# Changfei-Fu/RUMI-SLAM

Measured on AMD Instinct MI355X. Metric: frames/sec ORB extract+match, higher is better.
Workload: dtype u8; 1 GPU; ORB extract (640x480, 8-level pyramid, 1000 features/frame) + brute-force 256-bit Hamming match of consecutive frames (BASELINE.json configs[1]+[2]); scaling=n/a (one GPU), exchange=none

## Files before the change

include/rumi_testhooks.h:

```cpp
#ifndef RUMI_TESTHOOKS_H
#define RUMI_TESTHOOKS_H
#include <stdint.h>
#ifdef __cplusplus
extern "C" {
#endif

int rumi_hook_sort_like_std(uint32_t *keys, uint16_t *ids, int32_t n);
int rumi_hook_sort_device(uint32_t *keys, uint16_t *ids, int32_t n);
int rumi_hook_std_sort(uint32_t *keys, uint16_t *ids, int32_t n);

int rumi_hook_quadtree(const uint32_t *cand, int32_t n, int32_t minX, int32_t maxX, int32_t minY, int32_t maxY,
                       int32_t N, int32_t *out_idx, int32_t cap, int32_t *n_out);

float rumi_hook_sinf(float x);
float rumi_hook_cosf(float x);
float rumi_hook_fast_atan2(float y, float x);
int rumi_hook_cv_round(float v);
int rumi_hook_magic_div(int32_t idx, int32_t d);

struct RumiMatcher;
int rumi_hook_newpts_matches(struct RumiMatcher *m, int32_t n_neigh, int32_t n1, int32_t *matches);

#ifdef __cplusplus
}
#endif
#endif
```

rumi_slam_amd/capi.py:

```python
import ctypes as C
import os

import numpy as np

_HERE = os.path.dirname(os.path.abspath(__file__))
LIB_PATH = os.path.join(_HERE, "librumi_hip.so")

RUMI_OK, RUMI_E_INVALID, RUMI_E_NO_DEVICE, RUMI_E_CAPACITY, RUMI_E_EMPTY = 0, -1, -2, -3, -4

KP_DTYPE = np.dtype([("x", "<f4"), ("y", "<f4"), ("size", "<f4"), ("angle", "<f4"),
                     ("response", "<f4"), ("octave", "<i4"), ("class_id", "<i4")])
assert KP_DTYPE.itemsize == 28


class RumiOrbConfig(C.Structure):
    _fields_ = [("nfeatures", C.c_int32), ("scale_factor", C.c_float), ("nlevels", C.c_int32),
                ("ini_th_fast", C.c_int32), ("min_th_fast", C.c_int32), ("max_width", C.c_int32),
                ("max_height", C.c_int32), ("max_batch", C.c_int32), ("device", C.c_int32),
                ("host_threads", C.c_int32), ("blur_variant", C.c_int32)]


class RumiError(RuntimeError):
    def __init__(self, code, msg):
        super().__init__(f"rumi status {code}: {msg}")
# ... 77 lines not shown


def kfdb_lib():
    L = lib()
    if getattr(L, "_kfdb_ready", False):
        return L
    vp, i32, i64, u64 = C.c_void_p, C.c_int32, C.c_int64, C.c_uint64
    L.rumi_kfdb_create.argtypes = [vp, i32, i64, i32, C.POINTER(vp)]
    L.rumi_kfdb_destroy.argtypes = [vp]
    L.rumi_kfdb_destroy.restype = None
    L.rumi_kfdb_clear.argtypes = [vp]
    L.rumi_kfdb_size.argtypes = [vp]
    L.rumi_kfdb_next_seq.argtypes = [vp]
    L.rumi_kfdb_next_seq.restype = i64
    L.rumi_kfdb_max_batch.argtypes = [vp]
    L.rumi_kfdb_add.argtypes = [vp, i32, vp, vp, vp, vp, vp]
    L.rumi_kfdb_add_batch_device.argtypes = [vp, i32, vp, vp, vp, vp, vp, i32, vp]
    L.rumi_kfdb_bow.argtypes = [vp, u64, vp, vp, i32, C.POINTER(i32)]
    L.rumi_kfdb_erase.argtypes = [vp, i32, vp]
    L.rumi_kfdb_clear_map.argtypes = [vp, i32]
    L.rumi_kfdb_set_map_bad.argtypes = [vp, i32, i32]
    L.rumi_kfdb_set_maps.argtypes = [vp, i32, vp, vp]
    L.rumi_kfdb_set_bad.argtypes = [vp, i32, vp, vp]
    L.rumi_kfdb_set_covisibles.argtypes = [vp, i32, vp, vp]
    L.rumi_kfdb_score.argtypes = [vp, i32, i32, vp, vp, vp, vp, vp, vp, vp, vp, vp]
    L.rumi_kfdb_scored.argtypes = [vp, vp, vp]
    L.rumi_kfdb_select_reloc.argtypes = [vp, vp, vp, i64]
    L.rumi_kfdb_select_nbest.argtypes = [vp, vp, i32, vp, vp, vp, vp]
    L._kfdb_ready = True
    return L


HOOK_SYMBOLS = ["rumi_hook_sort_like_std", "rumi_hook_sort_device", "rumi_hook_std_sort", "rumi_hook_quadtree", "rumi_hook_sinf", "rumi_hook_cosf",
                "rumi_hook_fast_atan2", "rumi_hook_cv_round", "rumi_hook_magic_div", "rumi_hook_newpts_matches"]


def hooks():
    L = lib()
    if getattr(L, "_hooks_ready", False):
        return L
    vp, i32 = C.c_void_p, C.c_int32
    L.rumi_hook_sort_like_std.argtypes = [vp, vp, i32]
    L.rumi_hook_sort_device.argtypes = [vp, vp, i32]
    L.rumi_hook_std_sort.argtypes = [vp, vp, i32]
    L.rumi_hook_quadtree.argtypes = [vp, i32, i32, i32, i32, i32, i32, vp, i32, C.POINTER(i32)]
    for name in ("rumi_hook_sinf", "rumi_hook_cosf"):
        getattr(L, name).restype = C.c_float
        getattr(L, name).argtypes = [C.c_float]
    L.rumi_hook_fast_atan2.restype = C.c_float
    L.rumi_hook_fast_atan2.argtypes = [C.c_float, C.c_float]
    L.rumi_hook_cv_round.argtypes = [C.c_float]
    L.rumi_hook_magic_div.argtypes = [i32, i32]
    L._hooks_ready = True
    return L
```

rumi_slam_amd/csrc/orb_geom.h:

```cpp
#pragma once
#include <algorithm>
#include <cfloat>
#include <cmath>
#include <cstdint>
#include <vector>

namespace rumi {

constexpr int kPatchSize = 31;
constexpr int kHalfPatch = 15;
constexpr int kEdge = 19;
constexpr int kBorder = kEdge - 3;
constexpr int kMaxLevels = 16;
constexpr int kCellTileMax = 96;

inline int cv_round_host(double v) { return (int)std::lrint(v); }

#if defined(__HIPCC__)
#define RUMI_GEOM_HD __host__ __device__ inline
#else
#define RUMI_GEOM_HD inline
#endif
RUMI_GEOM_HD unsigned magic_of(unsigned d) { return (1u << 20) / d + 1u; }
RUMI_GEOM_HD int magic_div(int idx, unsigned M) { return (int)(((unsigned)idx * M) >> 20); }
// ... 55 lines not shown
inline bool make_geometry(const OrbTables &t, int w, int h, std::vector<LevelGeom> &g,
                          long long *arenaBytes, int *totalCells, int *totalCand, int *maxCellCand) {
    g.assign(t.nlevels, LevelGeom{});
    long long off = 0;
    int cells = 0, cand = 0, cellCand = 1;
    for (int l = 0; l < t.nlevels; l++) {
        LevelGeom &L = g[l];
        L.w = cv_round_host((float)w * t.invScale[l]);
        L.h = cv_round_host((float)h * t.invScale[l]);
        L.pitch = (L.w + 63) & ~63;
        L.off = off;
        off += (long long)L.pitch * L.h + 64;
        L.maxBX = L.w - kBorder; L.maxBY = L.h - kBorder;
        const float width = (float)(L.maxBX - kBorder), height = (float)(L.maxBY - kBorder);
        L.nCols = (int)(width / 35.f); L.nRows = (int)(height / 35.f);
        if (L.nCols <= 0 || L.nRows <= 0) return false;
        L.wCell = (int)std::ceil(width / L.nCols); L.hCell = (int)std::ceil(height / L.nRows);
        if (L.wCell + 6 > kCellTileMax || L.hCell + 6 > kCellTileMax) return false;
        L.cellBase = cells; L.nCells = L.nCols * L.nRows; cells += L.nCells;
        L.nfeat = t.featuresPerLevel[l];
        L.scale = t.scale[l];
        const int dw = L.maxBX - kBorder - 6, dh = L.maxBY - kBorder - 6;
        L.candBase = cand;
        L.candCap = std::min(65535, std::max(1, ((dw + 1) / 2) * ((dh + 1) / 2)));
        cand += L.candCap;
        cellCand = std::max(cellCand, ((L.wCell + 1) / 2) * ((L.hCell + 1) / 2));
        L.coefOff = 0;
    }
    *arenaBytes = (off + 255) & ~255LL;
    *totalCells = cells; *totalCand = cand; *maxCellCand = cellCand;
    return true;
}

inline void make_resize_axis(int srcN, int dstN, bool clampX, std::vector<int16_t> &ofs,
                             std::vector<int16_t> &taps, int *maxOut) {
    const double inv = (double)dstN / srcN, scale = 1. / inv;
    ofs.resize(dstN); taps.resize(dstN * 2);
    int dmax = dstN;
    for (int d = 0; d < dstN; d++) {
        float f = (float)((d + 0.5) * scale - 0.5);
        int s = (int)std::floor(f);
        f -= s;
        if (clampX) {
            if (s < 0) { f = 0; s = 0; }
            if (s + 1 >= srcN) {
                dmax = std::min(dmax, d);
                if (s >= srcN - 1) { f = 0; s = srcN - 1; }
            }
        }
        ofs[d] = (int16_t)s;
        taps[d * 2] = (int16_t)cv_round_host((1.f - f) * 2048.f);
        taps[d * 2 + 1] = (int16_t)cv_round_host(f * 2048.f);
    }
    *maxOut = dmax;
}

}
```

rumi_slam_amd/csrc/orb_kernels.hip:

```cpp
#include <hip/hip_runtime.h>

#include "orb_device.h"
#include "orb_math.h"

namespace rumi {

struct PatternF { float v[256 * 4]; };
constexpr PatternF make_pattern_f() {
    constexpr int8_t src[256 * 4] = {
#include "orb_pattern.inc"
    };
    PatternF p{};
    for (int i = 0; i < 256 * 4; i++) p.v[i] = (float)src[i];
    return p;
}
__constant__ PatternF c_patternF = make_pattern_f();

__device__ __forceinline__ unsigned xcd_swizzle(unsigned lin, unsigned total) {
    const unsigned q = total >> 3, r = total & 7, xcd = lin & 7;
    return (xcd < r ? xcd * (q + 1) : r * (q + 1) + (xcd - r) * q) + (lin >> 3);
}

struct __attribute__((packed)) U32 { uint32_t v; };
struct __attribute__((packed)) U64 { uint64_t v; };
constexpr int kPyrLevels = 8, kPyrWinPasses = 20;

__device__ __forceinline__ const uint8_t *level_base(const ImgSrc &s, const DevParams *P, int level, int frame,
                                                      int *pitch) {
    if (level == 0) {
        *pitch = s.l0Pitch;
        return s.l0 + (long long)frame * s.l0FrameStride;
    }
    *pitch = P->lv[level].pitch;
    return s.pyr + (long long)frame * P->arenaStride + P->lv[level].off;
}

__device__ __forceinline__ int reflect101(int i, int n) {
    if (n == 1) return 0;
    while (i < 0 || i >= n) i = i < 0 ? -i : 2 * (n - 1) - i;
    return i;
}

template <int kResizeRows>
__global__ __launch_bounds__(256) void k_resize(const DevParams *__restrict__ P, ImgSrc src,
                                                const int16_t *__restrict__ coef, const RowTap *__restrict__ rowTab, int level, int32_t *__restrict__ clearWord) {
    if (clearWord && (blockIdx.x | blockIdx.y | blockIdx.z | threadIdx.x) == 0) *clearWord = 0;
    const DevLevel &D = P->lv[level];
    const DevLevel &S = P->lv[level - 1];
    const unsigned wg = xcd_swizzle((blockIdx.z * gridDim.y + blockIdx.y) * gridDim.x + blockIdx.x, gridDim.x * gridDim.y * gridDim.z);
    const int bx = wg % gridDim.x, by = (wg / gridDim.x) % gridDim.y, frame = wg / (gridDim.x * gridDim.y);
    const int ox = (bx * 64 + (threadIdx.x & 63)) * 4;
    const int oyBase = (by * 4 + __builtin_amdgcn_readfirstlane(threadIdx.x >> 6)) * kResizeRows;
    if (ox >= D.w || oyBase >= D.h) return;
    int sp;
    const uint8_t *sb = level_base(src, P, level - 1, frame, &sp);
    uint8_t *dbase = src.pyr + (long long)frame * P->arenaStride + D.off + ox;
    const int16_t *xofs = coef + D.coefX, *xa = coef + D.coefXT;
    const uint8_t *r0p[kResizeRows], *r1p[kResizeRows];
    uint32_t bh0[kResizeRows], bh1[kResizeRows];
    bool live[kResizeRows], shared[kResizeRows];
#pragma unroll
    for (int r = 0; r < kResizeRows; r++) {
        const int oy = oyBase + r;
        live[r] = oy < D.h;
        const RowTap t = rowTab[D.rowTab + (live[r] ? oy : 0)];
        r0p[r] = sb + (long long)t.r0 * sp; r1p[r] = sb + (long long)t.r1 * sp;
        bh0[r] = t.bh0; bh1[r] = t.bh1;
        shared[r] = kResizeRows == 4 && r > 0 && r0p[r] == r1p[r - 1];
    }
    const int sx0 = xofs[ox];
    if (ox + 3 < D.xmaxFast && xofs[ox + 3] + 1 - sx0 <= 7) {
        const int wx0 = min(sx0, S.w - 8);
        const uint64_t ofs = reinterpret_cast<const U64 *>(xofs + ox)->v;
        const U64 *t8 = reinterpret_cast<const U64 *>(xa + 2 * ox);
        const uint64_t ta = t8[0].v, tb = t8[1].v;
        uint64_t s0[kResizeRows], s1[kResizeRows];
#pragma unroll
        for (int r = 0; r < kResizeRows; r++) {
            s0[r] = 0;
            if (!shared[r]) s0[r] = reinterpret_cast<const U64 *>(r0p[r] + wx0)->v;
            s1[r] = reinterpret_cast<const U64 *>(r1p[r] + wx0)->v;
        }
        typedef unsigned short v2u16 __attribute__((ext_vector_type(2)));
        uint32_t sel[4], tap[4];
#pragma unroll
        for (int i = 0; i < 4; i++) {
            const uint32_t k = (uint32_t)((int)(int16_t)(ofs >> (16 * i)) - wx0);
            sel[i] = k | 0x0c000c00u | ((k + 1u) << 16);
            const uint64_t tt = i < 2 ? ta : tb;
            tap[i] = (uint32_t)(tt >> (32 * (i & 1)));
        }
        uint32_t hPrev[4] = {0, 0, 0, 0};
#pragma unroll
        for (int r = 0; r < kResizeRows; r++) {
            uint32_t h0[4], h1[4];
            if (shared[r]) {
#pragma unroll
                for (int i = 0; i < 4; i++) h0[i] = hPrev[i];
            } else {
#pragma unroll
                for (int i = 0; i < 4; i++) {
                    const uint32_t p0 = __builtin_amdgcn_perm((uint32_t)(s0[r] >> 32), (uint32_t)s0[r], sel[i]);
                    h0[i] = __builtin_amdgcn_udot2(__builtin_bit_cast(v2u16, p0), __builtin_bit_cast(v2u16, tap[i]), 0u, false) >> 4;
                }
            }
            uint32_t packed = 0;
#pragma unroll
            for (int i = 0; i < 4; i++) {
                const uint32_t p1 = __builtin_amdgcn_perm((uint32_t)(s1[r] >> 32), (uint32_t)s1[r], sel[i]);
                h1[i] = __builtin_amdgcn_udot2(__builtin_bit_cast(v2u16, p1), __builtin_bit_cast(v2u16, tap[i]), 0u, false) >> 4;
                packed |= ((__umulhi(bh0[r], h0[i]) + __umulhi(bh1[r], h1[i]) + 2u) >> 2) << (8 * i);
                hPrev[i] = h1[i];
            }
            if (live[r]) *reinterpret_cast<uint32_t *>(dbase + (long long)(oyBase + r) * D.pitch) = packed;
        }
    } else {
        for (int r = 0; r < kResizeRows; r++) {
            if (!live[r]) continue;
            uint32_t packed = 0;
            for (int i = 0; i < 4 && ox + i < D.w; i++) {
                const int dx = ox + i;
                const int sx = xofs[dx];
                int q0, q1;
                if (dx < D.xmax) {
                    const int a0 = xa[dx * 2], a1 = xa[dx * 2 + 1];
                    q0 = r0p[r][sx] * a0 + r0p[r][sx + 1] * a1;
                    q1 = r1p[r][sx] * a0 + r1p[r][sx + 1] * a1;
                } else {
                    q0 = r0p[r][sx] * 2048;
                    q1 = r1p[r][sx] * 2048;
                }
                packed |= (uint32_t)(((((int)(bh0[r] >> 16) * (q0 >> 4)) >> 16) + (((int)(bh1[r] >> 16) * (q1 >> 4)) >> 16) + 2) >> 2) << (8 * i);
            }
            *reinterpret_cast<uint32_t *>(dbase + (long long)(oyBase + r) * D.pitch) = packed;
        }
    }
}

__global__ __launch_bounds__(256) void k_pyramid_tiles(const DevParams *__restrict__ P, ImgSrc src, const int16_t *__restrict__ coef,
                                                       const RowTap *__restrict__ rowTab, const PyrTile *__restrict__ tiles, int bufBytes,
                                                       int32_t *__restrict__ clearWord) {
    extern __shared__ __attribute__((aligned(16))) uint8_t pyrLds[];
    if (clearWord && (blockIdx.x | blockIdx.y | threadIdx.x) == 0) *clearWord = 0;
    const int frame = blockIdx.y, tid = threadIdx.x, nlevels = P->nlevels;
    uint8_t *A = pyrLds, *B = pyrLds + bufBytes;
    uint2 *tab = reinterpret_cast<uint2 *>(pyrLds + 2 * bufBytes);
    struct Lv { int x0, x1, y0, y1, coefX, coefXT, xmax, rowTab, pitch, pad; long long off; };
    __shared__ Lv sLv[kMaxLevels];
    if (tid < nlevels) {
        const PyrTile &T = tiles[blockIdx.x];
        const DevLevel &D = P->lv[tid];
        sLv[tid] = Lv{T.x0[tid], T.x1[tid], T.y0[tid], T.y1[tid], D.coefX, D.coefXT, D.xmax, D.rowTab, D.pitch, 0, D.off};
    }
    __syncthreads();
    int apitch;
// ... 501 lines not shown
    }
    if (tid == 0) sStart[nc] = total;
    int run = base + inc - sum;
    for (int k = 0; k < chunk; k++) {
        const int c = tid * chunk + k;
        if (c < nc) { sStart[c] = run; run += cnt[c]; }
    }
    __syncthreads();
    int32_t *ls = levelStart + (long long)frame * (kMaxLevels + 1);
    if (blockIdx.y == 0 && tid <= P->nlevels) {
        const int c = tid < P->nlevels ? P->lv[tid].cellBase : nc;
        ls[tid] = sStart[c];
    }
    if (blockIdx.y == 0 && tid < P->nlevels) {
        const int c0 = P->lv[tid].cellBase, c1 = c0 + P->lv[tid].nCells;
        if (sStart[c1] - sStart[c0] > P->lv[tid].candCap) atomicOr(errFlag, 16);
    }
    uint32_t *out = cand + (long long)frame * P->totalCand;
    const int nOut = min(sStart[nc], P->totalCand);
    const uint32_t *inBase = cellBuf + (long long)frame * nc * P->maxCellCand;
    for (int j = blockIdx.y * kCompactThreads + tid; j < nOut; j += kCompactThreads * gridDim.y) {
        int lo = 0, hi = nc;
        while (hi - lo > 1) {
            const int mid = (lo + hi) >> 1;
            if (sStart[mid] <= j) lo = mid; else hi = mid;
        }
        out[j] = inBase[(long long)lo * P->maxCellCand + (j - sStart[lo])];
    }
}

constexpr int kBlurRowsSmall = 16, kBlurRowsBatch = 64;

struct BlurGrid { int base[kMaxLevels + 1]; int gx[kMaxLevels]; int bw[kMaxLevels]; };
__device__ __forceinline__ uint32_t mad_u24(uint32_t a, uint32_t b, uint32_t c) {
    uint32_t r;
    asm("v_mad_u32_u24 %0, %1, %2, %3" : "=v"(r) : "v"(a), "v"(b), "v"(c));
    return r;
}
template <int VARIANT, int kBlurRows>
__device__ __forceinline__ void blur_body(const DevParams *__restrict__ P, const ImgSrc &src, const BlurGrid &G, unsigned bxg, unsigned gxg) {
    constexpr uint32_t kT2 = VARIANT ? 49u : 48u, kT3 = VARIANT ? 55u : 56u;
    const int lane = threadIdx.x & 63, wave = __builtin_amdgcn_readfirstlane(threadIdx.x >> 6);
    const unsigned wg = xcd_swizzle(blockIdx.y * gxg + bxg, gxg * gridDim.y);
    const int frame = wg / gxg, lin = wg % gxg;
    int level = 0;
    for (int l = 1; l < P->nlevels; l++)
        if (lin >= G.base[l]) level = l;
    const DevLevel &L = P->lv[level];
    const int bx = (lin - G.base[level]) % G.gx[level], by = (lin - G.base[level]) / G.gx[level];
    const int bw = G.bw[level];
    const int xa = bx * bw + lane * 4;
    const int y0 = (by * 4 + wave) * kBlurRows;
    if (y0 >= L.h) return;
    int pitch;
    const uint8_t *img = level_base(src, P, level, frame, &pitch);
    uint8_t *out = src.blur + (long long)frame * P->arenaStride + L.off;
    const int w = L.w, h = L.h;
    const int xLast = (w - 1) & ~3;
    const int xl = min(xa, xLast);
    const bool firstBlock = bx == 0;
    const bool edgeWave = bx * bw + bw + 4 > w;
    const bool produce = lane * 4 < bw && xa < w;
    uint32_t selA = 0x03020100u, selB = 0x07060504u;
    if (edgeWave && xa + 3 >= w && xa <= xLast + 4) {
#pragma unroll
        for (int i = 0; i < 4; i++) {
            const int x = xa + i;
            if (x < w) continue;
            const int sx = 2 * (w - 1) - x, d = (xa - (sx & ~3)) >> 2;
            const uint32_t a = (d == 1 ? 4u : 0u) + (uint32_t)(sx & 3);
            const uint32_t b = d == 0 ? 4u + (uint32_t)(sx & 3) : (uint32_t)i;
            selA = (selA & ~(0xFFu << (8 * i))) | (a << (8 * i));
            selB = (selB & ~(0xFFu << (8 * i))) | (b << (8 * i));
        }
    }
    int ring[7][4];
#pragma unroll
    for (int k = 0; k < 7; k++)
#pragma unroll
        for (int i = 0; i < 4; i++) ring[k][i] = 0;
    const int yEnd = min(y0 + kBlurRows, h), rEnd = yEnd + 3;
    uint8_t *orow = out + (long long)(y0 - 6) * L.pitch + xa - L.pitch;
    const int haloOff = lane == 0 ? (firstBlock ? 0 : -4) : (lane == 63 && !edgeWave && bw == 256 ? 4 : 0);
    uint32_t Cn[7], Hn[7];
    auto fetch = [&](int r, uint32_t &C, uint32_t &H) {
        const int rc = min(r, rEnd - 1);
        const int rr = rc < 0 ? -rc : (rc >= h ? 2 * (h - 1) - rc : rc);
        const uint8_t *row = img + (long long)rr * pitch + xl;
        C = *reinterpret_cast<const uint32_t *>(row);
        H = 0;
        if (haloOff) H = *reinterpret_cast<const uint32_t *>(row + haloOff);
    };
#pragma unroll
    for (int j = 0; j < 7; j++) fetch(y0 - 3 + j, Cn[j], Hn[j]);
    uint32_t Cm[7], Hm[7];
    auto walk7 = [&](const uint32_t (&Cc)[7], const uint32_t (&Hc)[7], int r0) {
#pragma unroll
        for (int j = 0; j < 7; j++) {
            const int r = r0 + j;
            if (r >= rEnd) break;
            orow += L.pitch;
            uint32_t C = Cc[j];
            if (edgeWave) {
                const uint32_t c1 = __shfl_up(C, 1), c2 = __shfl_up(c1, 1);
                C = __builtin_amdgcn_perm(C, __builtin_amdgcn_perm(c1, c2, selA), selB);
            }
            uint32_t Lw = __shfl_up(C, 1), Rw = __shfl_down(C, 1);
            if (lane == 0) Lw = firstBlock ? __builtin_amdgcn_perm(C, C, 0x01020300u) : Hc[j];
            if (lane == 63 && !edgeWave && bw == 256) Rw = Hc[j];
            constexpr uint32_t tA = 18u | (34u << 8) | (kT2 << 16) | (kT3 << 24), tB = kT2 | (34u << 8) | (18u << 16);
            const uint32_t A0 = __builtin_amdgcn_alignbyte(C, Lw, 1), A1 = __builtin_amdgcn_alignbyte(C, Lw, 2), A2 = __builtin_amdgcn_alignbyte(C, Lw, 3);
            const uint32_t B0 = __builtin_amdgcn_alignbyte(Rw, C, 1), B1 = __builtin_amdgcn_alignbyte(Rw, C, 2), B2 = __builtin_amdgcn_alignbyte(Rw, C, 3);
            ring[j][0] = (int)__builtin_amdgcn_udot4(B0, tB, __builtin_amdgcn_udot4(A0, tA, 0u, false), false);
            ring[j][1] = (int)__builtin_amdgcn_udot4(B1, tB, __builtin_amdgcn_udot4(A1, tA, 0u, false), false);
            ring[j][2] = (int)__builtin_amdgcn_udot4(B2, tB, __builtin_amdgcn_udot4(A2, tA, 0u, false), false);
            ring[j][3] = (int)__builtin_amdgcn_udot4(Rw, tB, __builtin_amdgcn_udot4(C, tA, 0u, false), false);
            const int y = r - 3;
            if (y >= y0 && produce) {
                uint32_t o[4];
#pragma unroll
                for (int i = 0; i < 4; i++) {
                    uint32_t acc = mad_u24(kT3, (uint32_t)ring[(j + 4) % 7][i], 32768u);
                    acc = mad_u24(kT2, (uint32_t)(ring[(j + 3) % 7][i] + ring[(j + 5) % 7][i]), acc);
                    acc = mad_u24(34u, (uint32_t)(ring[(j + 2) % 7][i] + ring[(j + 6) % 7][i]), acc);
                    acc = mad_u24(18u, (uint32_t)(ring[(j + 1) % 7][i] + ring[j][i]), acc);
                    if (VARIANT) acc = min(acc, 0x00FFFFFFu);
                    o[i] = acc;
                }
                const uint32_t p01 = __builtin_amdgcn_perm(o[1], o[0], 0x0c0c0602u), p23 = __builtin_amdgcn_perm(o[3], o[2], 0x06020c0cu);
                *reinterpret_cast<uint32_t *>(orow) = p01 | p23;
            }
        }
    };
    for (int r0 = y0 - 3; r0 < rEnd; r0 += 7) {
#pragma unroll
        for (int j = 0; j < 7; j++) Cm[j] = Cn[j], Hm[j] = Hn[j];
        if (r0 + 7 < rEnd) {
#pragma unroll
            for (int j = 0; j < 7; j++) fetch(r0 + 7 + j, Cn[j], Hn[j]);
        }
        walk7(Cm, Hm, r0);
    }
}
template <int VARIANT, int kBlurRows>
__global__ __launch_bounds__(256) void k_blur(const DevParams *__restrict__ P, ImgSrc src, BlurGrid G) {
    blur_body<VARIANT, kBlurRows>(P, src, G, blockIdx.x, gridDim.x);
}
template <int TPC, int VARIANT>
__global__ __launch_bounds__(256) void k_fast_blur(const DevParams *__restrict__ P, ImgSrc src, FastLds F, uint32_t *__restrict__ cellBuf,
                                                   int32_t *__restrict__ cellCnt, BlurGrid G, unsigned gxFast) {
    if (blockIdx.x < gxFast) fast_cells_body<TPC>(P, src, F, cellBuf, cellCnt, blockIdx.x, gxFast);
    else blur_body<VARIANT, kBlurRowsSmall>(P, src, G, blockIdx.x - gxFast, gridDim.x - gxFast);
}

__device__ __forceinline__ int half_wave_sum(int v) {
    v += __builtin_amdgcn_update_dpp(0, v, 0x111, 0xF, 0xF, false);
    v += __builtin_amdgcn_update_dpp(0, v, 0x112, 0xF, 0xF, false);
    v += __builtin_amdgcn_update_dpp(0, v, 0x114, 0xF, 0xF, false);
    v += __builtin_amdgcn_update_dpp(0, v, 0x118, 0xF, 0xF, false);
    v += __builtin_amdgcn_update_dpp(0, v, 0x142, 0xA, 0xF, false);
    const int lo = __builtin_amdgcn_readlane(v, 31), hi = __builtin_amdgcn_readlane(v, 63);
    return (threadIdx.x & 32) ? hi : lo;
}
__device__ __forceinline__ int wave_sum(int v) {
#pragma unroll
    for (int o = 32; o > 0; o >>= 1) v += __shfl_xor(v, o);
    return v;
}

constexpr int kDiscP = 48, kPatchP = 48;
constexpr int kKpPerWg = 8;

struct AssembleArgs {
    const uint32_t *selLevel; const int32_t *selLevelCnt; int selLevelCap, lap0, lap1;
    int32_t *counts; long long countsStride; int32_t *errFlag, *errMirror;
    uint32_t *selPackedOut, *selMetaOut; int32_t *selCountOut;
};
template <int kKpGroups, bool kAssemble>
__global__ __launch_bounds__(256, 7) void k_orient_desc(const DevParams *__restrict__ P, ImgSrc src,
                                                     const uint32_t *__restrict__ selPacked,
                                                     const uint32_t *__restrict__ selMeta,
                                                     const int32_t *__restrict__ selCount, int selCap,
                                                     RumiKeyPoint *__restrict__ kpOut, long long kpStride, uint8_t *__restrict__ descOut,
                                                     long long descStride, int outCap, AssembleArgs A) {
    static_assert(kDiscP == kPatchP, "the disc and the patch share their rows");
// ... 198 lines not shown
    uint32_t pkC = 0, mtC = 0, pkN = 0, mtN = 0;
    if (liveC) key_rec(kb, pkC, mtC);
    if (liveN && kKpGroups > 1) key_rec(kb + kKpPerWg, pkN, mtN);
    if (kKpGroups == 1) liveN = false;
    Staged S;
    fetch_disc(pkC, mtC, liveC, S);
    fetch_patch(pkC, mtC, liveC, S);
#pragma unroll
    for (int g = 0; g < kKpGroups; g++) {
        if (!__any(liveC)) break;
        OD_STAMP(0);
        stage_disc(liveC, S);
        OD_STAMP(1);
        const int k2 = kb + (g + 2) * kKpPerWg;
        const bool liveNN = g + 2 < kKpGroups && k2 < cnt;
        uint32_t pkNN = 0, mtNN = 0;
        if (liveNN) key_rec(k2, pkNN, mtNN);
        if (g + 1 < kKpGroups) fetch_disc(pkN, mtN, liveN, S);
        OD_STAMP(2);
        float angle = 0.f;
        if (liveC) angle = orientation(pkC);
        stage_patch(liveC, S);
        if (g + 1 < kKpGroups) fetch_patch(pkN, mtN, liveN, S);
        if (liveC) describe(pkC, mtC, angle);
        OD_STAMP(3);
        pkC = pkN; mtC = mtN; liveC = liveN;
        pkN = pkNN; mtN = mtNN; liveN = liveNN;
    }
#ifdef RUMI_OD_STAMP
    if (threadIdx.x == 0 && (blockIdx.x % 8) == 0 && blockIdx.y == 0) printf("od wg %d: loop-head %lld stage(wait loads) %lld issue-next %lld | IC_Angle %lld trig %lld rBRIEF %lld store %lld\n", (int)blockIdx.x, st[0], st[1], st[2], st[4], st[5], st[6], st[3]);
#endif
}

void launch_resize(const DevParams *dP, const DevParams &hP, ImgSrc src, const int16_t *coef, const RowTap *rowTab, int level, int nframes,
                   hipStream_t st, int32_t *clearWord) {
    const int rows = hP.lv[level].h >= 200 ? 8 : 4;
    dim3 g((hP.lv[level].w + 255) / 256, (hP.lv[level].h + 4 * rows - 1) / (4 * rows), nframes);
    if (rows == 8) hipLaunchKernelGGL(k_resize<8>, g, dim3(256), 0, st, dP, src, coef, rowTab, level, clearWord);
    else hipLaunchKernelGGL(k_resize<4>, g, dim3(256), 0, st, dP, src, coef, rowTab, level, clearWord);
}
void launch_pyramid_tiles(const DevParams *dP, ImgSrc src, const int16_t *coef, const RowTap *rowTab, const PyrTile *tiles, int ntiles, int bufBytes,
                          int tabEntries, int nframes, hipStream_t st, int32_t *clearWord) {
    hipLaunchKernelGGL(k_pyramid_tiles, dim3(ntiles, nframes), dim3(256), (size_t)2 * bufBytes + (size_t)tabEntries * 8, st, dP, src, coef, rowTab, tiles, bufBytes, clearWord);
}
static FastLds fast_lds_of(const DevParams &hP) {
    int wMax = 0, hMax = 0;
    for (int l = 0; l < hP.nlevels; l++) { wMax = std::max(wMax, hP.lv[l].wCell); hMax = std::max(hMax, hP.lv[l].hCell); }
    FastLds F;
    F.tp = 4 * (((wMax + 3) >> 2) + 2);
    F.sp = F.tp;
    F.tileBytes = (hMax + 6) * F.tp;
    F.scBytes = ((hMax + 2) * F.sp + 15) & ~15;
    F.maxIters = (wMax * hMax + 63) / 64 + 1;
    F.tileBytes = (F.tileBytes + 15) & ~15;
    F.perWave = (F.tileBytes + F.scBytes + std::max(kRingCap * 2, F.maxIters * 8) + kScoredCap * 2 + 15) & ~15;
    return F;
}
void launch_fast(const DevParams *dP, const DevParams &hP, ImgSrc src, uint32_t *cellBuf, int32_t *cellCnt, int nframes,
                 hipStream_t st) {
    const FastLds F = fast_lds_of(hP);
    const int wpg = 4;
    const dim3 grid((hP.totalCells + wpg - 1) / wpg, nframes);
    const size_t lds = (size_t)wpg * F.perWave;
#define RUMI_FAST_CASE(T)                                                                                      \
    if (F.tp == T) {                                                                                           \
        hipLaunchKernelGGL((k_fast_cells<T>), grid, dim3(64 * wpg), lds, st, dP, src, F, cellBuf, cellCnt);    \
        return;                                                                                                \
    }
    RUMI_FAST_CASE(48) RUMI_FAST_CASE(44) RUMI_FAST_CASE(52) RUMI_FAST_CASE(56)
#undef RUMI_FAST_CASE
    hipLaunchKernelGGL((k_fast_cells<0>), grid, dim3(64 * wpg), lds, st, dP, src, F, cellBuf, cellCnt);
}
// ... 9 lines not shown
        const bool partialInFirstLanes = r >= 1 && r <= 8;
        const bool lane63Halo = bw == 256 && (r >= 253 || r <= 3);
        if (!partialInFirstLanes && !lane63Halo) return bw;
    }
    return 192;
}
static BlurGrid blur_grid_of(const DevParams &hP, int rows, int *total) {
    BlurGrid G{};
    int run = 0;
    for (int l = 0; l < hP.nlevels; l++) {
        G.bw[l] = blur_strip_width(hP.lv[l].w);
        G.gx[l] = (hP.lv[l].w + G.bw[l] - 1) / G.bw[l];
        G.base[l] = run;
        run += G.gx[l] * ((hP.lv[l].h + 4 * rows - 1) / (4 * rows));
    }
    G.base[hP.nlevels] = run;
    *total = run;
    return G;
}
bool fast_blur_fusable(const DevParams &hP) { return fast_lds_of(hP).tp == 48; }
bool launch_fast_blur(const DevParams *dP, const DevParams &hP, ImgSrc src, uint32_t *cellBuf, int32_t *cellCnt, int nframes, int variant, hipStream_t st) {
    const FastLds F = fast_lds_of(hP);
    if (F.tp != 48) return false;
    int run = 0;
    const BlurGrid G = blur_grid_of(hP, kBlurRowsSmall, &run);
    const int wpg = 4;
    const unsigned gxFast = (unsigned)((hP.totalCells + wpg - 1) / wpg);
    const dim3 grid(gxFast + (unsigned)run, nframes);
    const size_t lds = (size_t)wpg * F.perWave;
    if (variant) hipLaunchKernelGGL((k_fast_blur<48, 1>), grid, dim3(256), lds, st, dP, src, F, cellBuf, cellCnt, G, gxFast);
    else hipLaunchKernelGGL((k_fast_blur<48, 0>), grid, dim3(256), lds, st, dP, src, F, cellBuf, cellCnt, G, gxFast);
    return true;
}
void launch_blur(const DevParams *dP, const DevParams &hP, ImgSrc src, int nframes, int variant, hipStream_t st) {
    const bool small = nframes < 16;
    const int rows = small ? kBlurRowsSmall : kBlurRowsBatch;
    int run = 0;
    const BlurGrid G = blur_grid_of(hP, rows, &run);
    if (small) {
        if (variant) hipLaunchKernelGGL((k_blur<1, kBlurRowsSmall>), dim3(run, nframes), dim3(256), 0, st, dP, src, G);
        else hipLaunchKernelGGL((k_blur<0, kBlurRowsSmall>), dim3(run, nframes), dim3(256), 0, st, dP, src, G);
    } else {
        if (variant) hipLaunchKernelGGL((k_blur<1, kBlurRowsBatch>), dim3(run, nframes), dim3(256), 0, st, dP, src, G);
        else hipLaunchKernelGGL((k_blur<0, kBlurRowsBatch>), dim3(run, nframes), dim3(256), 0, st, dP, src, G);
    }
}
void launch_orient_desc(const DevParams *dP, ImgSrc src, const uint32_t *selPacked, const uint32_t *selMeta,
                        const int32_t *selCount, int selCap, int maxSel, RumiKeyPoint *kpOut, long long kpStride, uint8_t *descOut,
                        long long descStride, int outCap, int nframes, hipStream_t st) {
    if (maxSel <= 0) return;
    const int wg1 = (maxSel + kKpPerWg - 1) / kKpPerWg;
    const AssembleArgs none{};
    if ((long long)wg1 * nframes <= 2048)
        hipLaunchKernelGGL((k_orient_desc<1, false>), dim3(wg1, nframes), dim3(256), 0, st, dP, src, selPacked, selMeta, selCount, selCap, kpOut, kpStride, descOut,
                           descStride, outCap, none);
    else
        hipLaunchKernelGGL((k_orient_desc<2, false>), dim3((wg1 + 1) / 2, nframes), dim3(256), 0, st, dP, src, selPacked, selMeta, selCount, selCap, kpOut, kpStride,
                           descOut, descStride, outCap, none);
}
void launch_assemble_orient_desc(const DevParams *dP, ImgSrc src, const uint32_t *selLevel, const int32_t *selLevelCnt, int selLevelCap, int lap0, int lap1,
                                 int32_t *counts, long long countsStride, int32_t *errFlag, int32_t *errMirror, uint32_t *selPacked, uint32_t *selMeta,
                                 int32_t *selCount, int selCap, int maxSel, RumiKeyPoint *kpOut,
                                 long long kpStride, uint8_t *descOut, long long descStride, int outCap, int nframes, hipStream_t st) {
    if (maxSel <= 0) return;
    const int wg1 = (maxSel + kKpPerWg - 1) / kKpPerWg;
    const AssembleArgs A{selLevel, selLevelCnt, selLevelCap, lap0, lap1, counts, countsStride, errFlag, nframes == 1 ? errMirror : nullptr, selPacked, selMeta, selCount};
    hipLaunchKernelGGL((k_orient_desc<1, true>), dim3(wg1, nframes), dim3(256), 0, st, dP, src, (const uint32_t *)nullptr, (const uint32_t *)nullptr,
                       (const int32_t *)nullptr, selCap, kpOut, kpStride, descOut, descStride, outCap, A);
}

}
```

rumi_slam_amd/csrc/testhooks.hip:

```cpp
#include <hip/hip_runtime.h>

#include <vector>

#include "orb_geom.h"
#include "orb_math.h"
#include "orb_octree.h"
#include "rumi_orb.h"
#include <algorithm>
#include <utility>
#include <vector>

#include "rumi_testhooks.h"

using namespace rumi;

extern "C" int rumi_hook_sort_like_std(uint32_t *keys, uint16_t *ids, int32_t n) {
    if (n < 0 || (n > 0 && (!keys || !ids))) return RUMI_E_INVALID;
    std::vector<OctEntry> e((size_t)n);
    for (int i = 0; i < n; i++) e[i] = OctEntry{keys[i], ids[i], 0};
    sort_like_libstdcxx(e.data(), n);
    for (int i = 0; i < n; i++) { keys[i] = e[i].key; ids[i] = e[i].id; }
    return RUMI_OK;
}

namespace rumi { int launch_sort_hook(uint32_t *keys, uint16_t *ids, int n); }
extern "C" int rumi_hook_sort_device(uint32_t *keys, uint16_t *ids, int32_t n) { return rumi::launch_sort_hook(keys, ids, n); }
extern "C" int rumi_hook_std_sort(uint32_t *keys, uint16_t *ids, int32_t n) {
    if (n < 0) return -1;
    std::vector<std::pair<uint32_t, uint16_t>> v(n);
    for (int i = 0; i < n; i++) v[i] = {keys[i], ids[i]};
    std::sort(v.begin(), v.end(), [](const std::pair<uint32_t, uint16_t> &a, const std::pair<uint32_t, uint16_t> &b) { return a.first < b.first; });
    for (int i = 0; i < n; i++) { keys[i] = v[i].first; ids[i] = v[i].second; }
    return 0;
}

extern "C" int rumi_hook_quadtree(const uint32_t *cand, int32_t n, int32_t minX, int32_t maxX, int32_t minY,
                                  int32_t maxY, int32_t N, int32_t *out_idx, int32_t cap, int32_t *n_out) {
    if (!n_out || n < 0 || n > 65535 || maxX <= minX || maxY <= minY) return RUMI_E_INVALID;
    std::vector<int> out;
    int m = octree_host(cand, n, minX, maxX, minY, maxY, N, out);
    if (m < 0) return RUMI_E_INVALID;
    *n_out = m;
    if (m > cap) return RUMI_E_CAPACITY;
    for (int i = 0; i < m; i++) out_idx[i] = out[i];
    return RUMI_OK;
}

extern "C" float rumi_hook_sinf(float x) { return sinf_glibc(x); }
extern "C" float rumi_hook_cosf(float x) { return cosf_glibc(x); }
extern "C" float rumi_hook_fast_atan2(float y, float x) { return fast_atan2_deg(y, x); }
extern "C" int rumi_hook_cv_round(float v) { return cv_round_f(v); }
extern "C" int rumi_hook_magic_div(int32_t idx, int32_t d) { return magic_div(idx, magic_of((unsigned)d)); }
```

Before: 291,200 frames/s.

## Pack multiple frames' narrow pyramid rows into shared wavefront lanes for resize and blur

Resize and blur kernels now map wavefront lanes across several frames' rows (lane packing with group size G up to 8), so narrow upper pyramid levels no longer leave most of a 64-lane wave idle. A magic-multiply divide maps each lane to a frame and column. The packed blur uses a 62-lane stride with one halo lane on each side instead of separate halo loads, and it handles frame seams with a ballot. This cuts the number of issued waves for batched workloads at the cost of extra index arithmetic, 32-bit offset limits, and a new kernel variant, with a test hook added for validation.

After: 309,200 frames/s (median of 6 runs). 6.2% higher.

```diff
diff --git a/include/rumi_testhooks.h b/include/rumi_testhooks.h
--- a/include/rumi_testhooks.h
+++ b/include/rumi_testhooks.h
@@ -18,6 +18,9 @@
 int rumi_hook_cv_round(float v);
 int rumi_hook_magic_div(int32_t idx, int32_t d);
 
+int rumi_hook_lane_packing(int32_t w, int32_t h, float scale, int32_t nlevels, int32_t nframes, int32_t kernel, int32_t level, int32_t force_g,
+                           int32_t *info, int32_t *slots, int32_t cap, int32_t *n_out);
+
 struct RumiMatcher;
 int rumi_hook_newpts_matches(struct RumiMatcher *m, int32_t n_neigh, int32_t n1, int32_t *matches);
 
diff --git a/rumi_slam_amd/capi.py b/rumi_slam_amd/capi.py
--- a/rumi_slam_amd/capi.py
+++ b/rumi_slam_amd/capi.py
@@ -133,7 +133,7 @@
 
 
 HOOK_SYMBOLS = ["rumi_hook_sort_like_std", "rumi_hook_sort_device", "rumi_hook_std_sort", "rumi_hook_quadtree", "rumi_hook_sinf", "rumi_hook_cosf",
-                "rumi_hook_fast_atan2", "rumi_hook_cv_round", "rumi_hook_magic_div", "rumi_hook_newpts_matches"]
+                "rumi_hook_fast_atan2", "rumi_hook_cv_round", "rumi_hook_magic_div", "rumi_hook_newpts_matches", "rumi_hook_lane_packing"]
 
 
 def hooks():
@@ -152,5 +152,6 @@
     L.rumi_hook_fast_atan2.argtypes = [C.c_float, C.c_float]
     L.rumi_hook_cv_round.argtypes = [C.c_float]
     L.rumi_hook_magic_div.argtypes = [i32, i32]
+    L.rumi_hook_lane_packing.argtypes = [i32, i32, C.c_float, i32, i32, i32, i32, i32, vp, vp, i32, C.POINTER(i32)]
     L._hooks_ready = True
     return L
diff --git a/rumi_slam_amd/csrc/orb_geom.h b/rumi_slam_amd/csrc/orb_geom.h
--- a/rumi_slam_amd/csrc/orb_geom.h
+++ b/rumi_slam_amd/csrc/orb_geom.h
@@ -111,6 +111,61 @@
     return true;
 }
 
+struct LanePack {
+    int lpr;
+    int halo;
+    int G;
+    int step, lead;
+    int waves;
+    unsigned M;
+};
+struct LaneSlot {
+    int frame, col;
+    bool live;
+    bool produce;
+    bool first;
+    bool last;
+};
+RUMI_GEOM_HD int lane_pack_waves(int lpr, int G, int step) { return (G * lpr + step - 1) / step; }
+RUMI_GEOM_HD LaneSlot lane_slot(const LanePack &K, int wave, int lane) {
+    const int v = wave * K.step - K.lead + lane;
+    const unsigned vv = v < 0 ? 0u : (unsigned)v;
+    LaneSlot s;
+    s.frame = (int)(((unsigned long long)vv * K.M) >> 32);
+    s.col = (int)vv - s.frame * K.lpr;
+    s.live = v >= 0 && s.frame < K.G;
+    s.produce = s.live && lane >= K.lead && lane < K.lead + K.step && s.col < K.lpr - K.halo;
+    s.first = s.col == 0;
+    s.last = s.col == K.lpr - 1;
+    return s;
+}
+RUMI_GEOM_HD int lane_frame(const LanePack &K, const LaneSlot &s, int group, int nframes) {
+    const int f = group * K.G + s.frame;
+    return s.live && f < nframes ? f : -1;
+}
+constexpr int kLanePackMaxG = 8;
+inline LanePack lane_pack_choose(int lpr, int halo, int step, int lead, int nframes, int maxG, long long spanBytes) {
+    LanePack K{lpr, halo, 1, step, lead, lane_pack_waves(lpr, 1, step), (unsigned)((1ull << 32) / (unsigned)lpr) + 1u};
+    long long best = (long long)nframes * K.waves;
+    for (int G = 2; G <= std::min(std::min(maxG, kLanePackMaxG), nframes); G++) {
+        if (spanBytes <= 0 || (long long)G * spanBytes >= (1ll << 31)) break;
+        if (((long long)G * lpr + 64) * lpr >= (1ll << 32)) break;
+        const int waves = lane_pack_waves(lpr, G, step);
+        const long long issued = (long long)((nframes + G - 1) / G) * waves;
+        if (issued < best) { best = issued; K.G = G; K.waves = waves; }
+    }
+    return K;
+}
+RUMI_GEOM_HD int resize_lanes_per_row(int w) { return (w + 3) >> 2; }
+RUMI_GEOM_HD int blur_lanes_per_row(int w) { return ((w + 3) >> 2) + 1; }
+constexpr int kPackMinFrames = 16;
+inline LanePack resize_pack_of(int w, int nframes, long long spanBytes) {
+    return lane_pack_choose(resize_lanes_per_row(w), 0, 64, 0, nframes, nframes >= kPackMinFrames ? kLanePackMaxG : 1, spanBytes);
+}
+inline LanePack blur_pack_of(int w, int nframes, long long spanBytes) {
+    return lane_pack_choose(blur_lanes_per_row(w), 1, 62, 1, nframes, kLanePackMaxG, spanBytes);
+}
+
 inline void make_resize_axis(int srcN, int dstN, bool clampX, std::vector<int16_t> &ofs,
                              std::vector<int16_t> &taps, int *maxOut) {
     const double inv = (double)dstN / srcN, scale = 1. / inv;
diff --git a/rumi_slam_amd/csrc/orb_kernels.hip b/rumi_slam_amd/csrc/orb_kernels.hip
--- a/rumi_slam_amd/csrc/orb_kernels.hip
+++ b/rumi_slam_amd/csrc/orb_kernels.hip
@@ -43,18 +43,21 @@
 
 template <int kResizeRows>
 __global__ __launch_bounds__(256) void k_resize(const DevParams *__restrict__ P, ImgSrc src,
-                                                const int16_t *__restrict__ coef, const RowTap *__restrict__ rowTab, int level, int32_t *__restrict__ clearWord) {
+                                                const int16_t *__restrict__ coef, const RowTap *__restrict__ rowTab, int level, int32_t *__restrict__ clearWord,
+                                                LanePack K, int nframes) {
     if (clearWord && (blockIdx.x | blockIdx.y | blockIdx.z | threadIdx.x) == 0) *clearWord = 0;
     const DevLevel &D = P->lv[level];
     const DevLevel &S = P->lv[level - 1];
     const unsigned wg = xcd_swizzle((blockIdx.z * gridDim.y + blockIdx.y) * gridDim.x + blockIdx.x, gridDim.x * gridDim.y * gridDim.z);
-    const int bx = wg % gridDim.x, by = (wg / gridDim.x) % gridDim.y, frame = wg / (gridDim.x * gridDim.y);
-    const int ox = (bx * 64 + (threadIdx.x & 63)) * 4;
+    const int bx = wg % gridDim.x, by = (wg / gridDim.x) % gridDim.y, group = wg / (gridDim.x * gridDim.y), frame0 = group * K.G;
+    const LaneSlot slot = lane_slot(K, bx, threadIdx.x & 63);
+    const int ox = slot.col * 4;
     const int oyBase = (by * 4 + __builtin_amdgcn_readfirstlane(threadIdx.x >> 6)) * kResizeRows;
-    if (ox >= D.w || oyBase >= D.h) return;
+    if (lane_frame(K, slot, group, nframes) < 0 || oyBase >= D.h) return;
     int sp;
-    const uint8_t *sb = level_base(src, P, level - 1, frame, &sp);
-    uint8_t *dbase = src.pyr + (long long)frame * P->arenaStride + D.off + ox;
+    const uint8_t *sb = level_base(src, P, level - 1, frame0, &sp);
+    const uint32_t fo = (uint32_t)slot.frame * (uint32_t)(level == 1 ? src.l0FrameStride : P->arenaStride);
+    uint8_t *dbase = src.pyr + (long long)frame0 * P->arenaStride + D.off + ((uint32_t)slot.frame * (uint32_t)P->arenaStride + (uint32_t)ox);
     const int16_t *xofs = coef + D.coefX, *xa = coef + D.coefXT;
     const uint8_t *r0p[kResizeRows], *r1p[kResizeRows];
     uint32_t bh0[kResizeRows], bh1[kResizeRows];
@@ -71,6 +74,7 @@
     const int sx0 = xofs[ox];
     if (ox + 3 < D.xmaxFast && xofs[ox + 3] + 1 - sx0 <= 7) {
         const int wx0 = min(sx0, S.w - 8);
+        const uint32_t wo = fo + (uint32_t)wx0;
         const uint64_t ofs = reinterpret_cast<const U64 *>(xofs + ox)->v;
         const U64 *t8 = reinterpret_cast<const U64 *>(xa + 2 * ox);
         const uint64_t ta = t8[0].v, tb = t8[1].v;
@@ -78,8 +82,8 @@
 #pragma unroll
         for (int r = 0; r < kResizeRows; r++) {
             s0[r] = 0;
-            if (!shared[r]) s0[r] = reinterpret_cast<const U64 *>(r0p[r] + wx0)->v;
-            s1[r] = reinterpret_cast<const U64 *>(r1p[r] + wx0)->v;
+            if (!shared[r]) s0[r] = reinterpret_cast<const U64 *>(r0p[r] + wo)->v;
+            s1[r] = reinterpret_cast<const U64 *>(r1p[r] + wo)->v;
         }
         typedef unsigned short v2u16 __attribute__((ext_vector_type(2)));
         uint32_t sel[4], tap[4];
@@ -120,7 +124,7 @@
             uint32_t packed = 0;
             for (int i = 0; i < 4 && ox + i < D.w; i++) {
                 const int dx = ox + i;
-                const int sx = xofs[dx];
+                const uint32_t sx = fo + (uint32_t)xofs[dx];
                 int q0, q1;
                 if (dx < D.xmax) {
                     const int a0 = xa[dx * 2], a1 = xa[dx * 2 + 1];
@@ -688,35 +692,54 @@
 constexpr int kBlurRowsSmall = 16, kBlurRowsBatch = 64;
 
 struct BlurGrid { int base[kMaxLevels + 1]; int gx[kMaxLevels]; int bw[kMaxLevels]; };
+struct BlurPack { int base[kMaxLevels + 1]; int gx[kMaxLevels], gy[kMaxLevels], G[kMaxLevels]; unsigned M[kMaxLevels]; int nframes; };
 __device__ __forceinline__ uint32_t mad_u24(uint32_t a, uint32_t b, uint32_t c) {
     uint32_t r;
     asm("v_mad_u32_u24 %0, %1, %2, %3" : "=v"(r) : "v"(a), "v"(b), "v"(c));
     return r;
 }
-template <int VARIANT, int kBlurRows>
-__device__ __forceinline__ void blur_body(const DevParams *__restrict__ P, const ImgSrc &src, const BlurGrid &G, unsigned bxg, unsigned gxg) {
+template <int VARIANT, int kBlurRows, bool kPacked, typename Grid>
+__device__ __forceinline__ void blur_body(const DevParams *__restrict__ P, const ImgSrc &src, const Grid &G, unsigned bxg, unsigned gxg) {
     constexpr uint32_t kT2 = VARIANT ? 49u : 48u, kT3 = VARIANT ? 55u : 56u;
     const int lane = threadIdx.x & 63, wave = __builtin_amdgcn_readfirstlane(threadIdx.x >> 6);
-    const unsigned wg = xcd_swizzle(blockIdx.y * gxg + bxg, gxg * gridDim.y);
-    const int frame = wg / gxg, lin = wg % gxg;
+    const unsigned wg = kPacked ? xcd_swizzle(bxg, gxg) : xcd_swizzle(blockIdx.y * gxg + bxg, gxg * gridDim.y);
+    const int lin = kPacked ? wg : wg % gxg;
+    int frame = kPacked ? 0 : wg / gxg;
     int level = 0;
     for (int l = 1; l < P->nlevels; l++)
         if (lin >= G.base[l]) level = l;
     const DevLevel &L = P->lv[level];
-    const int bx = (lin - G.base[level]) % G.gx[level], by = (lin - G.base[level]) / G.gx[level];
-    const int bw = G.bw[level];
-    const int xa = bx * bw + lane * 4;
+    int bx, by, bw, xa;
+    uint32_t fsrc = 0, fdst = 0;
+    bool produce, first = false;
+    if constexpr (kPacked) {
+        const int per = G.gx[level] * G.gy[level], idx = lin - G.base[level], group = idx / per;
+        bx = (idx - group * per) % G.gx[level]; by = (idx - group * per) / G.gx[level];
+        frame = group * G.G[level];
+        const LanePack K{blur_lanes_per_row(L.w), 1, G.G[level], 62, 1, G.gx[level], G.M[level]};
+        const LaneSlot slot = lane_slot(K, bx, lane);
+        const bool mine = lane_frame(K, slot, group, G.nframes) >= 0;
+        const uint32_t f = mine ? (uint32_t)slot.frame : 0u;
+        fsrc = f * (uint32_t)(level == 0 ? src.l0FrameStride : P->arenaStride); fdst = f * (uint32_t)P->arenaStride;
+        bw = 256; xa = slot.col * 4;
+        produce = mine && slot.produce; first = slot.first;
+    } else {
+        bx = (lin - G.base[level]) % G.gx[level]; by = (lin - G.base[level]) / G.gx[level];
+        bw = G.bw[level];
+        xa = bx * bw + lane * 4;
+    }
     const int y0 = (by * 4 + wave) * kBlurRows;
     if (y0 >= L.h) return;
     int pitch;
     const uint8_t *img = level_base(src, P, level, frame, &pitch);
-    uint8_t *out = src.blur + (long long)frame * P->arenaStride + L.off;
+    uint8_t *out = src.blur + (long long)frame * P->arenaStride + L.off + fdst;
     const int w = L.w, h = L.h;
     const int xLast = (w - 1) & ~3;
     const int xl = min(xa, xLast);
     const bool firstBlock = bx == 0;
-    const bool edgeWave = bx * bw + bw + 4 > w;
-    const bool produce = lane * 4 < bw && xa < w;
+    const bool edgeWave = kPacked ? __builtin_amdgcn_ballot_w64(xa + 3 >= w) != 0 : bx * bw + bw + 4 > w;
+    const bool seamWave = kPacked && __builtin_amdgcn_ballot_w64(first) != 0;
+    if constexpr (!kPacked) produce = lane * 4 < bw && xa < w;
     uint32_t selA = 0x03020100u, selB = 0x07060504u;
     if (edgeWave && xa + 3 >= w && xa <= xLast + 4) {
 #pragma unroll
@@ -737,15 +760,16 @@
         for (int i = 0; i < 4; i++) ring[k][i] = 0;
     const int yEnd = min(y0 + kBlurRows, h), rEnd = yEnd + 3;
     uint8_t *orow = out + (long long)(y0 - 6) * L.pitch + xa - L.pitch;
-    const int haloOff = lane == 0 ? (firstBlock ? 0 : -4) : (lane == 63 && !edgeWave && bw == 256 ? 4 : 0);
+    const int haloOff = kPacked ? 0 : lane == 0 ? (firstBlock ? 0 : -4) : (lane == 63 && !edgeWave && bw == 256 ? 4 : 0);
     uint32_t Cn[7], Hn[7];
     auto fetch = [&](int r, uint32_t &C, uint32_t &H) {
         const int rc = min(r, rEnd - 1);
         const int rr = rc < 0 ? -rc : (rc >= h ? 2 * (h - 1) - rc : rc);
-        const uint8_t *row = img + (long long)rr * pitch + xl;
+        const uint8_t *row = img + (long long)rr * pitch;
+        if constexpr (kPacked) row += fsrc + (uint32_t)xl; else row += xl;
         C = *reinterpret_cast<const uint32_t *>(row);
         H = 0;
-        if (haloOff) H = *reinterpret_cast<const uint32_t *>(row + haloOff);
+        if (!kPacked && haloOff) H = *reinterpret_cast<const uint32_t *>(row + haloOff);
     };
 #pragma unroll
     for (int j = 0; j < 7; j++) fetch(y0 - 3 + j, Cn[j], Hn[j]);
@@ -762,8 +786,12 @@
                 C = __builtin_amdgcn_perm(C, __builtin_amdgcn_perm(c1, c2, selA), selB);
             }
             uint32_t Lw = __shfl_up(C, 1), Rw = __shfl_down(C, 1);
-            if (lane == 0) Lw = firstBlock ? __builtin_amdgcn_perm(C, C, 0x01020300u) : Hc[j];
-            if (lane == 63 && !edgeWave && bw == 256) Rw = Hc[j];
+            if constexpr (kPacked) {
+                if (seamWave && first) Lw = __builtin_amdgcn_perm(C, C, 0x01020300u);
+            } else {
+                if (lane == 0) Lw = firstBlock ? __builtin_amdgcn_perm(C, C, 0x01020300u) : Hc[j];
+                if (lane == 63 && !edgeWave && bw == 256) Rw = Hc[j];
+            }
             constexpr uint32_t tA = 18u | (34u << 8) | (kT2 << 16) | (kT3 << 24), tB = kT2 | (34u << 8) | (18u << 16);
             const uint32_t A0 = __builtin_amdgcn_alignbyte(C, Lw, 1), A1 = __builtin_amdgcn_alignbyte(C, Lw, 2), A2 = __builtin_amdgcn_alignbyte(C, Lw, 3);
             const uint32_t B0 = __builtin_amdgcn_alignbyte(Rw, C, 1), B1 = __builtin_amdgcn_alignbyte(Rw, C, 2), B2 = __builtin_amdgcn_alignbyte(Rw, C, 3);
@@ -800,13 +828,17 @@
 }
 template <int VARIANT, int kBlurRows>
 __global__ __launch_bounds__(256) void k_blur(const DevParams *__restrict__ P, ImgSrc src, BlurGrid G) {
-    blur_body<VARIANT, kBlurRows>(P, src, G, blockIdx.x, gridDim.x);
+    blur_body<VARIANT, kBlurRows, false>(P, src, G, blockIdx.x, gridDim.x);
+}
+template <int VARIANT>
+__global__ __launch_bounds__(256) void k_blur_packed(const DevParams *__restrict__ P, ImgSrc src, BlurPack G) {
+    blur_body<VARIANT, kBlurRowsBatch, true>(P, src, G, blockIdx.x, gridDim.x);
 }
 template <int TPC, int VARIANT>
 __global__ __launch_bounds__(256) void k_fast_blur(const DevParams *__restrict__ P, ImgSrc src, FastLds F, uint32_t *__restrict__ cellBuf,
                                                    int32_t *__restrict__ cellCnt, BlurGrid G, unsigned gxFast) {
     if (blockIdx.x < gxFast) fast_cells_body<TPC>(P, src, F, cellBuf, cellCnt, blockIdx.x, gxFast);
-    else blur_body<VARIANT, kBlurRowsSmall>(P, src, G, blockIdx.x - gxFast, gridDim.x - gxFast);
+    else blur_body<VARIANT, kBlurRowsSmall, false>(P, src, G, blockIdx.x - gxFast, gridDim.x - gxFast);
 }
 
 __device__ __forceinline__ int half_wave_sum(int v) {
@@ -1071,12 +1103,17 @@
 #endif
 }
 
+static long long pack_span(const DevParams &hP, const ImgSrc &src, bool readsLevel0) {
+    if (readsLevel0 && src.l0FrameStride <= 0) return 0;
+    return readsLevel0 ? std::max(hP.arenaStride, src.l0FrameStride) : hP.arenaStride;
+}
 void launch_resize(const DevParams *dP, const DevParams &hP, ImgSrc src, const int16_t *coef, const RowTap *rowTab, int level, int nframes,
                    hipStream_t st, int32_t *clearWord) {
     const int rows = hP.lv[level].h >= 200 ? 8 : 4;
-    dim3 g((hP.lv[level].w + 255) / 256, (hP.lv[level].h + 4 * rows - 1) / (4 * rows), nframes);
-    if (rows == 8) hipLaunchKernelGGL(k_resize<8>, g, dim3(256), 0, st, dP, src, coef, rowTab, level, clearWord);
-    else hipLaunchKernelGGL(k_resize<4>, g, dim3(256), 0, st, dP, src, coef, rowTab, level, clearWord);
+    const LanePack K = resize_pack_of(hP.lv[level].w, nframes, pack_span(hP, src, level == 1));
+    dim3 g(K.waves, (hP.lv[level].h + 4 * rows - 1) / (4 * rows), (nframes + K.G - 1) / K.G);
+    if (rows == 8) hipLaunchKernelGGL(k_resize<8>, g, dim3(256), 0, st, dP, src, coef, rowTab, level, clearWord, K, nframes);
+    else hipLaunchKernelGGL(k_resize<4>, g, dim3(256), 0, st, dP, src, coef, rowTab, level, clearWord, K, nframes);
 }
 void launch_pyramid_tiles(const DevParams *dP, ImgSrc src, const int16_t *coef, const RowTap *rowTab, const PyrTile *tiles, int ntiles, int bufBytes,
                           int tabEntries, int nframes, hipStream_t st, int32_t *clearWord) {
@@ -1152,18 +1189,32 @@
     else hipLaunchKernelGGL((k_fast_blur<48, 0>), grid, dim3(256), lds, st, dP, src, F, cellBuf, cellCnt, G, gxFast);
     return true;
 }
+static BlurPack blur_pack_grid(const DevParams &hP, int nframes, long long span, int *total) {
+    BlurPack G{};
+    int run = 0;
+    for (int l = 0; l < hP.nlevels; l++) {
+        const LanePack K = blur_pack_of(hP.lv[l].w, nframes, span);
+        G.gx[l] = K.waves; G.gy[l] = (hP.lv[l].h + 4 * kBlurRowsBatch - 1) / (4 * kBlurRowsBatch); G.G[l] = K.G; G.M[l] = K.M;
+        G.base[l] = run;
+        run += G.gx[l] * G.gy[l] * ((nframes + K.G - 1) / K.G);
+    }
+    G.base[hP.nlevels] = run;
+    G.nframes = nframes;
+    *total = run;
+    return G;
+}
 void launch_blur(const DevParams *dP, const DevParams &hP, ImgSrc src, int nframes, int variant, hipStream_t st) {
-    const bool small = nframes < 16;
-    const int rows = small ? kBlurRowsSmall : kBlurRowsBatch;
+    if (nframes >= kPackMinFrames) {
+        int run = 0;
+        const BlurPack G = blur_pack_grid(hP, nframes, pack_span(hP, src, true), &run);
+        if (variant) hipLaunchKernelGGL((k_blur_packed<1>), dim3(run), dim3(256), 0, st, dP, src, G);
+        else hipLaunchKernelGGL((k_blur_packed<0>), dim3(run), dim3(256), 0, st, dP, src, G);
+        return;
+    }
     int run = 0;
-    const BlurGrid G = blur_grid_of(hP, rows, &run);
-    if (small) {
-        if (variant) hipLaunchKernelGGL((k_blur<1, kBlurRowsSmall>), dim3(run, nframes), dim3(256), 0, st, dP, src, G);
-        else hipLaunchKernelGGL((k_blur<0, kBlurRowsSmall>), dim3(run, nframes), dim3(256), 0, st, dP, src, G);
-    } else {
-        if (variant) hipLaunchKernelGGL((k_blur<1, kBlurRowsBatch>), dim3(run, nframes), dim3(256), 0, st, dP, src, G);
-        else hipLaunchKernelGGL((k_blur<0, kBlurRowsBatch>), dim3(run, nframes), dim3(256), 0, st, dP, src, G);
-    }
+    const BlurGrid G = blur_grid_of(hP, kBlurRowsSmall, &run);
+    if (variant) hipLaunchKernelGGL((k_blur<1, kBlurRowsSmall>), dim3(run, nframes), dim3(256), 0, st, dP, src, G);
+    else hipLaunchKernelGGL((k_blur<0, kBlurRowsSmall>), dim3(run, nframes), dim3(256), 0, st, dP, src, G);
 }
 void launch_orient_desc(const DevParams *dP, ImgSrc src, const uint32_t *selPacked, const uint32_t *selMeta,
                         const int32_t *selCount, int selCap, int maxSel, RumiKeyPoint *kpOut, long long kpStride, uint8_t *descOut,
diff --git a/rumi_slam_amd/csrc/testhooks.hip b/rumi_slam_amd/csrc/testhooks.hip
--- a/rumi_slam_amd/csrc/testhooks.hip
+++ b/rumi_slam_amd/csrc/testhooks.hip
@@ -51,3 +51,33 @@
 extern "C" float rumi_hook_fast_atan2(float y, float x) { return fast_atan2_deg(y, x); }
 extern "C" int rumi_hook_cv_round(float v) { return cv_round_f(v); }
 extern "C" int rumi_hook_magic_div(int32_t idx, int32_t d) { return magic_div(idx, magic_of((unsigned)d)); }
+
+extern "C" int rumi_hook_lane_packing(int32_t w, int32_t h, float scale, int32_t nlevels, int32_t nframes, int32_t kernel, int32_t level,
+                                      int32_t force_g, int32_t *info, int32_t *slots, int32_t cap, int32_t *n_out) {
+    if (!info || !n_out || nframes < 1 || nlevels < 1 || nlevels > kMaxLevels || kernel < 0 || kernel > 1 || level < (kernel ? 0 : 1) || level >= nlevels ||
+        force_g < 0 || force_g > nframes)
+        return RUMI_E_INVALID;
+    const OrbTables t = make_tables(1000, scale, nlevels);
+    std::vector<LevelGeom> g;
+    long long arena = 0;
+    int cells, cand, cellCand;
+    if (!make_geometry(t, w, h, g, &arena, &cells, &cand, &cellCand)) return RUMI_E_INVALID;
+    const long long span = std::max(arena, (long long)w * h);
+    LanePack K = kernel ? blur_pack_of(g[level].w, nframes, span) : resize_pack_of(g[level].w, nframes, span);
+    if (force_g) { K.G = force_g; K.waves = lane_pack_waves(K.lpr, K.G, K.step); }
+    const int groups = (nframes + K.G - 1) / K.G;
+    const int32_t inf[8] = {g[level].w, K.lpr, K.G, K.waves, groups, K.step, K.halo, g[level].h};
+    std::copy(inf, inf + 8, info);
+    const long long n = (long long)groups * K.waves * 64;
+    *n_out = (int32_t)std::min<long long>(n, INT32_MAX);
+    if (n > cap || !slots) return RUMI_E_CAPACITY;
+    int32_t *o = slots;
+    for (int grp = 0; grp < groups; grp++)
+        for (int wv = 0; wv < K.waves; wv++)
+            for (int lane = 0; lane < 64; lane++, o += 3) {
+                const LaneSlot s = lane_slot(K, wv, lane);
+                const int f = lane_frame(K, s, grp, nframes);
+                o[0] = f; o[1] = s.col; o[2] = (f >= 0 && s.produce ? 1 : 0) | (s.first ? 2 : 0) | (s.last ? 4 : 0);
+            }
+    return RUMI_OK;
+}
```
